# ap229997/hands

Hardware: AMD Instinct MI355X
Metric: hands/sec (higher is better)
Workload: dtype f32; 1 GPU; hands_light ResNet-50 x3 + feature_conv + HMR + MANO, 224x224, bz=256 samples/GPU (512 hands, 768 trunk passes); per_gpu_batch=256, global_batch=256, parallelism=dp1, rccl_ranks=1, launched_by=direct, conv3x3_stride1=winograd_f4x4:stages1234

## Files before the change

hands_amd/csrc/conv_wino4.hip:

```cpp
#include <hip/hip_runtime.h>
#include <stdint.h>
#include <stdlib.h>
#include "hands_hip.h"
#include "common.h"

#ifdef W4_PROF
__device__ unsigned long long g_w4prof[512 * 2 * 64];
extern "C" int hands_debug_w4prof(void* dst, int clear) {
  hipDeviceSynchronize();
  if (dst) hipMemcpyFromSymbol(dst, HIP_SYMBOL(g_w4prof), sizeof(unsigned long long) * 512 * 2 * 64);
  if (clear) { static unsigned long long z[512 * 2 * 64]; hipMemcpyToSymbol(HIP_SYMBOL(g_w4prof), z, sizeof(z)); }
  return 0;
}
#define W4_STAMP(ROLE, IDX)                                                                          \
  do {                                                                                              \
    __builtin_amdgcn_sched_barrier(0);                                                              \
    if (lane == 0 && blockIdx.x < 512 && (IDX) < 64 && (wave == 0 || wave == 12))                   \
      g_w4prof[(blockIdx.x * 2 + (ROLE)) * 64 + (IDX)] = __builtin_amdgcn_s_memtime();              \
    __builtin_amdgcn_sched_barrier(0);                                                              \
  } while (0)
#else
#define W4_STAMP(ROLE, IDX) do {} while (0)
#endif

namespace {

typedef unsigned int u32x4 __attribute__((ext_vector_type(4)));
typedef __attribute__((address_space(3))) void lds_void_t;

struct Wino4Args {
  const float* __restrict__ in;
  const float* __restrict__ u;
  const float* __restrict__ bias;
  float* out;
  int B, H, W, Cin, Cout, nh, nw;
  int in_ps, out_ps, act;
  int nblk_m, nblk_n, nseg;
  int band;
  int rows;
  uint32_t nh_mul, nh_sh;
};

__device__ __forceinline__ int w4_fastdiv(int x, uint32_t mul, uint32_t sh) {
  return mul == 0 ? x : (int)(__umulhi((uint32_t)x, mul) >> sh);
}

__device__ __forceinline__ int w4_xcd_remap(int bid, int nwg) {
  const int q = nwg >> 3, r = nwg & 7;
  const int xcd = bid & 7, idx = bid >> 3;
  const int base = (xcd < r) ? xcd * (q + 1) : r * (q + 1) + (xcd - r) * q;
  return base + idx;
}

__device__ __forceinline__ float4 w4_f4(const u32x4& v) {
  return make_float4(__uint_as_float(v.x), __uint_as_float(v.y), __uint_as_float(v.z), __uint_as_float(v.w));
}
__device__ __forceinline__ float w4_e(const float4& v, int t) { return t == 0 ? v.x : (t == 1 ? v.y : (t == 2 ? v.z : v.w)); }

__device__ __forceinline__ void w4_dma16(__amdgpu_buffer_rsrc_t rsrc, char* dst, int voff, int soff) {
  __builtin_amdgcn_raw_ptr_buffer_load_lds(rsrc, (lds_void_t*)dst, 16, voff, soff, 0, 0);
}

__device__ __forceinline__ void w4_bt6(const float (&x)[6], float (&v)[6]) {
  const float a = fmaf(-4.f, x[2], x[4]);
  const float b = fmaf(-4.f, x[1], x[3]);
  const float c = x[4] - x[2];
  const float d = x[3] - x[1];
  v[0] = fmaf(4.f, x[0], fmaf(-5.f, x[2], x[4]));
  v[1] = a + b;
  v[2] = a - b;
  v[3] = fmaf(2.f, d, c);
  v[4] = fmaf(-2.f, d, c);
  v[5] = fmaf(4.f, x[1], fmaf(-5.f, x[3], x[5]));
}

template <int D, bool LINEAR>
struct W4Geom {
  static constexpr int PW = 4 * D + 2;
  static constexpr int PWP = (PW + 3) / 4 * 4;
  static constexpr int NR = LINEAR ? (D - 1 + 32 + D - 1) / D : 32 / D;
  static constexpr int ROW_BYTES = PWP * 32;
  static constexpr int SLOTS = NR * 6 * PWP * 2;
  static constexpr int PIECES = (SLOTS + 63) / 64;
  static constexpr int NJ = (PIECES + 3) / 4;
  static constexpr int PATCH_BYTES = PIECES * 1024;
};

constexpr int W4_VBUF = 36 * 1024;
constexpr int W4_PATCH_MAX = 36 * 1024;
constexpr long long W4_BAND_BYTES = 2560 * 1024;

template <int D, bool LINEAR, int VSH>
__device__ __forceinline__ void w4_output_pass(const Wino4Args& a, const char* lds, int wave, int lane, int nb, int R0, int s0, int tx0) {
  constexpr int VM = (1 << VSH) - 1;
  const int rd = wave >> 2, oj = wave & 3;
  const int otl = lane >> 1, ocq = lane & 1;
  const int oqq = s0 + otl;
  const int oRl = LINEAR ? oqq / D : otl / D, ocol = LINEAR ? oqq - oRl * D : otl - oRl * D;
  const int oV = R0 + oRl, oR = oV >> VSH, otx = tx0 + (oV & VM) * D + ocol;
  const int ob = w4_fastdiv(oR, a.nh_mul, a.nh_sh), oty = oR - ob * a.nh;
  if (!(oR < a.rows && otx < a.nw && 4 * otx + oj < a.W)) return;
  const int n_ch = nb * 32 + rd * 8 + ocq * 4;
  float* const o = a.out + (((size_t)ob * a.H + 4 * oty) * a.W + 4 * otx + oj) * (size_t)a.out_ps + n_ch;
  const char* sE = lds + rd * W4_VBUF + otl * 32 + ocq * 16;
  const float kq = oj == 0 ? 1.f : (oj == 1 ? 2.f : (oj == 2 ? 4.f : 8.f));
  const int pi = (oj == 0 ? 0 : (oj == 2 ? 2 : 1)) * 1024, qi = (oj == 0 || oj == 2 ? 3 : 4) * 1024;
  float4 y[4];
#pragma unroll
  for (int x6 = 0; x6 < 6; ++x6) {
    const char* eb = sE + x6 * 6 * 1024;
    const float4 p0 = *reinterpret_cast<const float4*>(eb + pi);
    const float4 q0 = *reinterpret_cast<const float4*>(eb + qi);
    float4 z = make_float4(fmaf(kq, q0.x, p0.x), fmaf(kq, q0.y, p0.y), fmaf(kq, q0.z, p0.z), fmaf(kq, q0.w, p0.w));
    if (oj == 3) {
      const float4 m5 = *reinterpret_cast<const float4*>(eb + 5 * 1024);
      z.x += m5.x; z.y += m5.y; z.z += m5.z; z.w += m5.w;
    }
#define W4_ACC(C)                                                                                    \
    if (x6 == 0) { y[0].C = z.C; }                                                                  \
    else if (x6 == 1) { y[0].C += z.C; y[1].C = z.C; y[2].C = z.C; y[3].C = z.C; }                  \
    else if (x6 == 2) { y[0].C += z.C; y[1].C -= z.C; y[2].C += z.C; y[3].C -= z.C; }               \
    else if (x6 == 3) { y[0].C += z.C; y[1].C = fmaf(2.f, z.C, y[1].C); y[2].C = fmaf(4.f, z.C, y[2].C); y[3].C = fmaf(8.f, z.C, y[3].C); } \
    else if (x6 == 4) { y[0].C += z.C; y[1].C = fmaf(-2.f, z.C, y[1].C); y[2].C = fmaf(4.f, z.C, y[2].C); y[3].C = fmaf(-8.f, z.C, y[3].C); } \
    else { y[3].C += z.C; }
    W4_ACC(x) W4_ACC(y) W4_ACC(z) W4_ACC(w)
#undef W4_ACC
  }
  const float4 bv = *reinterpret_cast<const float4*>(a.bias + n_ch);
#pragma unroll
  for (int i = 0; i < 4; ++i) {
    float4 v = make_float4(y[i].x + bv.x, y[i].y + bv.y, y[i].z + bv.z, y[i].w + bv.w);
    if (a.act == HANDS_ACT_RELU) {
      v.x = fmaxf(v.x, 0.f); v.y = fmaxf(v.y, 0.f); v.z = fmaxf(v.z, 0.f); v.w = fmaxf(v.w, 0.f);
    } else if (a.act == HANDS_ACT_LEAKY_RELU) {
      v.x = v.x > 0.f ? v.x : 0.01f * v.x; v.y = v.y > 0.f ? v.y : 0.01f * v.y;
      v.z = v.z > 0.f ? v.z : 0.01f * v.z; v.w = v.w > 0.f ? v.w : 0.01f * v.w;
    }
    if (4 * oty + i < a.H) *reinterpret_cast<float4*>(o + (size_t)i * a.W * a.out_ps) = v;
  }
}

template <int D, bool LINEAR, int VSH, int NOB>
__global__ void __launch_bounds__(1024, 1) conv_wino4_f32_kernel(Wino4Args a) {
  using G = W4Geom<D, LINEAR>;
  static_assert(G::PATCH_BYTES <= W4_PATCH_MAX, "patch buffer");
  static_assert(VSH == 0 || LINEAR, "virtual rows exist in the linear block order only");
  __shared__ __attribute__((aligned(1024))) char lds[4 * W4_VBUF];
  char* const sV = lds;
  char* const sP = lds + 2 * W4_VBUF;

  const int tid = threadIdx.x;
  const int lane = tid & 63;
  const int wave = __builtin_amdgcn_readfirstlane(tid >> 6);
  const bool producer = wave >= 12;
  const int l31 = lane & 31, half = lane >> 5;
  constexpr int VM = (1 << VSH) - 1;

  const int wg = w4_xcd_remap(blockIdx.x, a.nblk_m * a.nblk_n);
  int nbg, mb;
  {
    const int full = a.nblk_n / a.band, per = a.band * a.nblk_m;
    int bi = wg / per, r = wg - bi * per, bw = a.band;
    if (bi >= full) { bi = full; r = wg - full * per; bw = a.nblk_n - full * a.band; }
    mb = r / bw;
    nbg = bi * a.band + (r - mb * bw);
  }
  const int nb = nbg * NOB;
  int R0, s0, tx0;
  if constexpr (LINEAR) {
    const int t0 = mb * 32;
    R0 = t0 / D; s0 = t0 - R0 * D; tx0 = 0;
  } else {
    const int rb = mb / a.nseg, seg = mb - rb * a.nseg;
    R0 = rb * G::NR; s0 = 0; tx0 = seg * D;
  }
  const int R0r = R0 >> VSH;
  const int b_first = w4_fastdiv(R0r, a.nh_mul, a.nh_sh);
  const int ty_first = R0r - b_first * a.nh;
  const int nsteps = a.Cin >> 3;

  if (producer) {
    W4_STAMP(1, 0);
    const int pw = wave - 12;
    __builtin_amdgcn_s_setprio(2);
    const __amdgpu_buffer_rsrc_t x_rsrc = __builtin_amdgcn_make_buffer_rsrc(
        const_cast<float*>(a.in) + (size_t)b_first * a.H * a.W * a.in_ps, 0, (int)0x80000000u, 0x00020000);
    int f_off[G::NJ];
#pragma unroll
    for (int j = 0; j < G::NJ; ++j) {
      const int i = j * 4 + pw;
      const int S = i * 64 + lane;
      const int r = S / (G::PWP * 2), within = S - r * (G::PWP * 2);
      const int Rl = r / 6, ar = r - Rl * 6;
      const int xg = within >> 3, sl = within & 7;
      const int swz = (D * Rl + xg) & 3;
      const int sl2 = sl ^ (swz << 1);
      const int x = 4 * xg + (sl2 >> 1), q = sl2 & 1;
      const int V = R0 + Rl, Rr = V >> VSH, pv = V & VM;
      const int t = ty_first + (Rr - R0r);
      const int db = w4_fastdiv(t, a.nh_mul, a.nh_sh), ty = t - db * a.nh;
      const int hy = 4 * ty - 1 + ar, wx = 4 * (tx0 + pv * D) - 1 + x;
      const bool ok = i < G::PIECES && x < G::PW && Rr < a.rows && (unsigned)hy < (unsigned)a.H && (unsigned)wx < (unsigned)a.W;
      f_off[j] = ok ? (((db * a.H + hy) * a.W + wx) * a.in_ps + q * 4) * 4 : (int)0x80000000u;
      if (i < G::PIECES) w4_dma16(x_rsrc, sP + i * 1024, f_off[j], 0);
    }
#define W4_PFILL(PB, G_)                                                                             \
  do {                                                                                              \
    _Pragma("unroll") for (int j = 0; j < G::NJ; ++j) {                                             \
      if (j * 4 + pw < G::PIECES) w4_dma16(x_rsrc, sP + (PB) * W4_VBUF + (j * 4 + pw) * 1024, f_off[j], (G_) * 32); \
    }                                                                                               \
  } while (0)
    if (nsteps > 1) W4_PFILL(1, 1);
    int tb[6];
    {
      const int tl = pw * 8 + (lane >> 3), c = lane & 7;
      const int qq = s0 + tl;
      const int Rl = LINEAR ? qq / D : tl / D, col = LINEAR ? qq - Rl * D : tl - Rl * D;
      const int swz0 = (D * Rl + col) & 3, swz1 = (swz0 + 1) & 3;
      const int q = c >> 2, w = c & 3;
#pragma unroll
      for (int b = 0; b < 6; ++b) {
        const int grp8 = b < 4 ? col : col + 1;
        const int sl = (2 * (b & 3) + q) ^ ((b < 4 ? swz0 : swz1) << 1);
        tb[b] = Rl * 6 * G::ROW_BYTES + (grp8 * 8 + sl) * 16 + w * 4;
      }
    }
    const int vw_off = pw * 256 + lane * 4;

#define W4_TRANSFORM(PB, VB, NEXT_FILL)                                                              \
  do {                                                                                              \
    const char* pp = sP + (PB) * W4_VBUF;                                                           \
    float xx[6][6];                                                                                 \
    _Pragma("unroll") for (int b = 0; b < 6; ++b)                                                   \
      _Pragma("unroll") for (int ar = 0; ar < 6; ++ar)                                              \
        xx[ar][b] = *reinterpret_cast<const float*>(pp + tb[b] + ar * G::ROW_BYTES);                \
    __builtin_amdgcn_sched_barrier(0);                                                              \
    NEXT_FILL;                                   \
    __builtin_amdgcn_sched_barrier(0);                                                              \
    float tt[6][6];                                                                                 \
    _Pragma("unroll") for (int b = 0; b < 6; ++b) {                                                 \
      float x[6], v[6];                                                                             \
      _Pragma("unroll") for (int ar = 0; ar < 6; ++ar) x[ar] = xx[ar][b];                           \
      w4_bt6(x, v);                                                                                 \
      _Pragma("unroll") for (int k = 0; k < 6; ++k) tt[k][b] = v[k];                                \
    }                                                                                               \
    char* vp = sV + (VB) * W4_VBUF + vw_off;                                                        \
    _Pragma("unroll") for (int k = 0; k < 6; ++k) {                                                 \
      float v[6];                                                                                   \
      w4_bt6(tt[k], v);                                                                             \
      _Pragma("unroll") for (int n = 0; n < 6; ++n) *reinterpret_cast<float*>(vp + (k * 6 + n) * 1024) = v[n]; \
    }                                                                                               \
  } while (0)

    __syncthreads();
    W4_TRANSFORM(0, 0, );
    __syncthreads();
    W4_STAMP(1, 1);
    for (int g = 0; g < nsteps; ++g) {
      W4_STAMP(1, 2 + 3 * g);
#if !(defined(W4_ABL) && W4_ABL == 2)
#if defined(W4_ABL) && W4_ABL == 5
      if (g + 1 < nsteps && (g & 2) == 0) {
#else
      if (g + 1 < nsteps) {
#endif
        if ((g & 1) == 0) W4_TRANSFORM(1, 1, if (g + 2 < nsteps) W4_PFILL(0, g + 2)); else W4_TRANSFORM(0, 0, if (g + 2 < nsteps) W4_PFILL(1, g + 2));
      }
#endif
      W4_STAMP(1, 3 + 3 * g);
      __syncthreads();
      W4_STAMP(1, 4 + 3 * g);
    }
#undef W4_TRANSFORM
#undef W4_PFILL
  }
  if (!producer) {
    W4_STAMP(0, 0);
    const int xi = wave >> 1, hh = wave & 1;
    const int f0 = xi * 6 + 3 * hh;
    const __amdgpu_buffer_rsrc_t w_rsrc = __builtin_amdgcn_make_buffer_rsrc(
        const_cast<float*>(a.u) + (size_t)nb * nsteps * 9216, 0, (int)0x80000000u, 0x00020000);
    const __amdgpu_buffer_rsrc_t w_rsrc1 = __builtin_amdgcn_make_buffer_rsrc(
        const_cast<float*>(a.u) + (size_t)(nb + NOB - 1) * nsteps * 9216, 0, (int)0x80000000u, 0x00020000);
    const int w_off = f0 * 1024 + lane * 16;
    const int v_off = f0 * 1024 + l31 * 32 + half * 16;
    f32x16 acc[3][NOB];
#pragma unroll
    for (int n = 0; n < 3; ++n)
#pragma unroll
      for (int o = 0; o < NOB; ++o)
#pragma unroll
        for (int r = 0; r < 16; ++r) acc[n][o][r] = 0.f;

    float4 wq[2][NOB], vq[2];
#define W4_LOADOP(SET, N, STEP, VP)                                                                  \
  do {                                                                                              \
    vq[SET] = *reinterpret_cast<const float4*>((VP) + (N) * 1024);                                  \
    wq[SET][0] = w4_f4(__builtin_amdgcn_raw_buffer_load_b128(w_rsrc, w_off + (N) * 1024, (STEP) * 36864, 0)); \
    if (NOB > 1) wq[SET][NOB - 1] = w4_f4(__builtin_amdgcn_raw_buffer_load_b128(w_rsrc1, w_off + (N) * 1024, (STEP) * 36864, 0)); \
  } while (0)
#define W4_LOADW(SET, N, STEP)                                                                       \
  do {                                                                                              \
    wq[SET][0] = w4_f4(__builtin_amdgcn_raw_buffer_load_b128(w_rsrc, w_off + (N) * 1024, (STEP) * 36864, 0)); \
    if (NOB > 1) wq[SET][NOB - 1] = w4_f4(__builtin_amdgcn_raw_buffer_load_b128(w_rsrc1, w_off + (N) * 1024, (STEP) * 36864, 0)); \
  } while (0)
#if defined(W4_ABL) && W4_ABL == 4
#define W4_NMFMA 1
#else
#define W4_NMFMA 4
#endif
#define W4_MFMAS(SET, N)                                                                             \
  do {                                                                                              \
    _Pragma("unroll") for (int o = 0; o < NOB; ++o)                                                 \
      _Pragma("unroll") for (int t = 0; t < W4_NMFMA; ++t)                                          \
        acc[N][o] = __builtin_amdgcn_mfma_f32_32x32x2f32(w4_e(wq[SET][o], t), w4_e(vq[SET], t), acc[N][o], 0, 0, 0); \
  } while (0)

#define W4_BARRIER() do { asm volatile("s_waitcnt lgkmcnt(0)\n\ts_barrier" ::: "memory"); } while (0)
    if constexpr (NOB == 2) {
#define W4_V2(N, VP) do { vq[0] = *reinterpret_cast<const float4*>((VP) + (N) * 1024); } while (0)
#define W4_MFMAS2(WSET, N)                                                                           \
  do {                                                                                              \
    _Pragma("unroll") for (int o = 0; o < NOB; ++o)                                                 \
      _Pragma("unroll") for (int t = 0; t < 4; ++t)                                                 \
        acc[N][o] = __builtin_amdgcn_mfma_f32_32x32x2f32(w4_e(wq[WSET][o], t), w4_e(vq[0], t), acc[N][o], 0, 0, 0); \
  } while (0)
      W4_LOADW(0, 0, 0);
      W4_BARRIER();
      W4_BARRIER();
      W4_STAMP(0, 1);
      for (int g = 0; g < nsteps; ++g) {
        const int gn = g + 1 < nsteps ? g + 1 : g;
        const char* vp = sV + (g & 1) * W4_VBUF + v_off;
        W4_V2(0, vp); W4_LOADW(1, 1, g);
        __builtin_amdgcn_sched_barrier(0);
        W4_MFMAS2(0, 0);
        __builtin_amdgcn_sched_barrier(0);
        W4_LOADW(0, 2, g);
        W4_V2(1, vp);
        __builtin_amdgcn_sched_barrier(0);
        W4_MFMAS2(1, 1);
        __builtin_amdgcn_sched_barrier(0);
        W4_V2(2, vp);
        __builtin_amdgcn_sched_barrier(0);
        W4_MFMAS2(0, 2);
        __builtin_amdgcn_sched_barrier(0);
        W4_LOADW(0, 0, gn);
        __builtin_amdgcn_sched_barrier(0);
        W4_STAMP(0, 2 + 3 * g);
        W4_BARRIER();
        W4_STAMP(0, 4 + 3 * g);
      }
#undef W4_MFMAS2
#undef W4_V2
    } else {
    W4_LOADW(0, 0, 0);
    W4_BARRIER();
    W4_BARRIER();
    W4_STAMP(0, 1);
    vq[0] = *reinterpret_cast<const float4*>(sV + v_off);
    for (int g = 0; g < nsteps; ++g) {
      const int gn = g + 1 < nsteps ? g + 1 : g;
      const char* vp = sV + (g & 1) * W4_VBUF + v_off;
      W4_LOADOP(1, 1, g, vp);
      __builtin_amdgcn_sched_barrier(0);
      W4_MFMAS(0, 0);
      __builtin_amdgcn_sched_barrier(0);
      W4_LOADOP(0, 2, g, vp);
      __builtin_amdgcn_sched_barrier(0);
      W4_MFMAS(1, 1);
      __builtin_amdgcn_sched_barrier(0);
      W4_LOADW(1, 0, gn);
      __builtin_amdgcn_sched_barrier(0);
      W4_MFMAS(0, 2);
      __builtin_amdgcn_sched_barrier(0);
      W4_STAMP(0, 2 + 3 * g);
      W4_BARRIER();
      W4_STAMP(0, 4 + 3 * g);
      {
        const char* vn = sV + ((g + 1) & 1) * W4_VBUF + v_off;
        vq[1] = *reinterpret_cast<const float4*>(vn);
      }
      if (++g >= nsteps) break;
      const int gn2 = g + 1 < nsteps ? g + 1 : g;
      const char* vp2 = sV + (g & 1) * W4_VBUF + v_off;
      W4_LOADOP(0, 1, g, vp2);
      __builtin_amdgcn_sched_barrier(0);
      W4_MFMAS(1, 0);
      __builtin_amdgcn_sched_barrier(0);
      W4_LOADOP(1, 2, g, vp2);
      __builtin_amdgcn_sched_barrier(0);
      W4_MFMAS(0, 1);
      __builtin_amdgcn_sched_barrier(0);
      W4_LOADW(0, 0, gn2);
      __builtin_amdgcn_sched_barrier(0);
      W4_MFMAS(1, 2);
      __builtin_amdgcn_sched_barrier(0);
      W4_STAMP(0, 2 + 3 * g);
      W4_BARRIER();
      W4_STAMP(0, 4 + 3 * g);
      vq[0] = *reinterpret_cast<const float4*>(sV + ((g + 1) & 1) * W4_VBUF + v_off);
    }
    }
#undef W4_BARRIER
#undef W4_LOADOP
#undef W4_LOADW
#undef W4_MFMAS

#define W4_LDS_BARRIER() do { asm volatile("s_waitcnt lgkmcnt(0)\n\ts_barrier" ::: "memory"); } while (0)
#pragma unroll
    for (int o = 0; o < NOB; ++o) {
      if (hh == 0) {
#pragma unroll
        for (int r = 0; r < 16; ++r) {
          const float s_ = acc[1][o][r] + acc[2][o][r], d_ = acc[1][o][r] - acc[2][o][r];
          acc[0][o][r] = acc[0][o][r] + s_; acc[1][o][r] = d_; acc[2][o][r] = s_;
        }
      } else {
#pragma unroll
        for (int r = 0; r < 16; ++r) {
          const float s_ = acc[0][o][r] + acc[1][o][r], d_ = acc[0][o][r] - acc[1][o][r];
          acc[0][o][r] = s_; acc[1][o][r] = d_;
        }
      }
      if (o > 0) W4_LDS_BARRIER();
#pragma unroll
      for (int rd = 0; rd < 4; ++rd)
#pragma unroll
        for (int n = 0; n < 3; ++n)
          *reinterpret_cast<float4*>(lds + rd * W4_VBUF + v_off + n * 1024) =
              make_float4(acc[n][o][4 * rd + 0], acc[n][o][4 * rd + 1], acc[n][o][4 * rd + 2], acc[n][o][4 * rd + 3]);
      if (NOB > 1) W4_LDS_BARRIER(); else __syncthreads();
      W4_STAMP(0, 60);
      w4_output_pass<D, LINEAR, VSH>(a, lds, wave, lane, nb + o, R0, s0, tx0);
    }
    W4_STAMP(0, 61);
    return;
  }
#pragma unroll
  for (int o = 0; o < NOB; ++o) {
    if (o > 0) W4_LDS_BARRIER();
    if (NOB > 1) W4_LDS_BARRIER(); else __syncthreads();
    W4_STAMP(1, 60);
    w4_output_pass<D, LINEAR, VSH>(a, lds, wave, lane, nb + o, R0, s0, tx0);
  }
  W4_STAMP(1, 61);
}

}

static void w4_magic(int d, uint32_t& mul, uint32_t& sh) {
  if (d <= 1) { mul = 0; sh = 0; return; }
  int l = 0;
  while ((1LL << l) < d) ++l;
  mul = (uint32_t)(((1ULL << (31 + l)) + (uint64_t)d - 1) / (uint64_t)d);
  sh = (uint32_t)(l - 1);
}

static long long w4_blocks(long long rows, int nw) {
  if (nw == 7 || nw == 14) return (rows * nw + 31) / 32;
  if (nw <= 2) return (rows + 15) / 16;
  return (rows + 7) / 8 * ((nw + 3) / 4);
}

template <int D, bool LINEAR, int VSH, int NOB>
static int w4_launch_nob(Wino4Args& a, hipStream_t stream) {
  using G = W4Geom<D, LINEAR>;
  const long long rows = a.rows;
  long long nblk_m;
  if (LINEAR) {
    nblk_m = (rows * (D << VSH) + 31) / 32;
    a.nseg = 1;
  } else {
    a.nseg = (a.nw + D - 1) / D;
    nblk_m = (rows + G::NR - 1) / G::NR * a.nseg;
  }
  a.nblk_n = a.Cout / (32 * NOB);
  {
    const long long wbytes = (long long)(a.Cin / 8) * 36864 * NOB;
    long long band = W4_BAND_BYTES / wbytes;
#ifdef HANDS_W4_BAND_ENV
    const char* env = getenv("HANDS_W4_BAND");
    if (env && atoi(env) > 0) band = atoi(env);
#endif
    a.band = (int)(band < 1 ? 1 : (band > a.nblk_n ? a.nblk_n : band));
  }
  if (nblk_m <= 0 || nblk_m * a.nblk_n > 0x7fffffffLL) return HANDS_EINVAL;
  a.nblk_m = (int)nblk_m;
  const long long nwg = nblk_m * a.nblk_n;
  w4_magic(a.nh, a.nh_mul, a.nh_sh);
  const long long imgs = G::NR / a.nh + 2;
  if (imgs * a.H * a.W * a.in_ps * 4 >= 0x7fffffffLL) return HANDS_EINVAL;
  hipLaunchKernelGGL((conv_wino4_f32_kernel<D, LINEAR, VSH, NOB>), dim3((unsigned)nwg), dim3(1024), 0, stream, a);
  return (int)hipGetLastError();
}

template <int D, bool LINEAR, int VSH = 0>
static int w4_launch(Wino4Args& a, hipStream_t stream) {
#ifndef HANDS_W4_NOB1
  if (a.Cout % 64 == 0) return w4_launch_nob<D, LINEAR, VSH, 2>(a, stream);
#endif
  return w4_launch_nob<D, LINEAR, VSH, 1>(a, stream);
}

static bool w4_ok(const hands_conv_desc* d) {
  if (d->B <= 0 || d->H <= 0 || d->W <= 0) return false;
  const int act = d->act & HANDS_ACT_MASK;
  const long long nh = (d->H + 3) / 4, nw = (d->W + 3) / 4, rows = (long long)d->B * nh;
  if (rows >= 0x7fffff00LL || rows * nw >= 0x7fffff00LL) return false;
  if (w4_blocks(rows, (int)nw) * (d->Cout / 32) > 0x7fffffffLL) return false;
  const long long ps = d->in_pix_stride > d->out_pix_stride ? d->in_pix_stride : d->out_pix_stride;
  if ((16 / nh + 2) * d->H * d->W * ps * 4 >= 0x7fffffffLL) return false;
  return d->KH == 3 && d->KW == 3 && d->stride == 1 && d->pad == 1 && d->Ho == d->H && d->Wo == d->W && d->Cin >= 16 &&
         d->Cin % 8 == 0 && d->Cout >= 32 && d->Cout % 32 == 0 && d->in_pix_stride >= d->Cin && d->out_pix_stride >= d->Cout &&
         d->in_pix_stride % 4 == 0 && d->out_pix_stride % 4 == 0 &&
         (act == HANDS_ACT_NONE || act == HANDS_ACT_RELU || act == HANDS_ACT_LEAKY_RELU) && !(d->act & HANDS_MATH_BF16X3);
}

extern "C" int hands_conv3x3_winograd4_supported(const hands_conv_desc* d) { return d && w4_ok(d) ? 1 : 0; }

extern "C" long long hands_conv3x3_winograd4_executed_macs(const hands_conv_desc* d) {
  if (!d || !w4_ok(d)) return 0;
  const long long nh = (d->H + 3) / 4, nw = (d->W + 3) / 4;
  return 36LL * w4_blocks((long long)d->B * nh, (int)nw) * 32 * d->Cin * d->Cout;
}

extern "C" int hands_conv3x3_winograd4_f32(const hands_conv_desc* d, const float* in, const float* u_packed, const float* bias,
                                           float* out, hands_stream_t stream) {
  if (!d || !in || !u_packed || !bias || !out || !w4_ok(d)) return HANDS_EINVAL;
  if ((((uintptr_t)in) | ((uintptr_t)u_packed) | ((uintptr_t)bias) | ((uintptr_t)out)) & 15) return HANDS_EINVAL;
  Wino4Args a;
  a.in = in; a.u = u_packed; a.bias = bias; a.out = out;
  a.B = d->B; a.H = d->H; a.W = d->W; a.Cin = d->Cin; a.Cout = d->Cout;
  a.nh = (d->H + 3) / 4; a.nw = (d->W + 3) / 4;
  a.in_ps = d->in_pix_stride; a.out_ps = d->out_pix_stride; a.act = d->act & HANDS_ACT_MASK;
  a.rows = d->B * a.nh;
  a.nblk_m = a.nblk_n = a.nseg = 0; a.band = 1;
  hipStream_t s = (hipStream_t)stream;
  if (a.nw == 7) return w4_launch<7, true>(a, s);
  if (a.nw == 14) return w4_launch<7, true, 1>(a, s);
  if (a.nw <= 2) return w4_launch<2, false>(a, s);
  return w4_launch<4, false>(a, s);
}
```

Baseline: 12090 hands/s.

## Spread Winograd F4 prologue patch DMA across all waves, use vmcnt-counted barriers

The initial input-patch loads for stage 0 are now issued by all 16 waves instead of only the 4 producer waves. The stage-1 prefetch is issued by the 12 consumer waves instead of the producers. The first two consumer barriers now wait on precise vmcnt counts, so the weight and stage-1 loads can stay in flight across the first barrier. Bias loads are hoisted ahead of the output-pass barriers, and the slot-offset math moves into a shared header. This is meant to shorten the prologue latency before the first MFMAs, at the cost of more complex wait accounting that could race if the counts are wrong.

```diff
diff --git a/hands_amd/csrc/conv_wino4.hip b/hands_amd/csrc/conv_wino4.hip
--- a/hands_amd/csrc/conv_wino4.hip
+++ b/hands_amd/csrc/conv_wino4.hip
@@ -3,6 +3,7 @@
 #include <stdlib.h>
 #include "hands_hip.h"
 #include "common.h"
+#include "wino4_slots.h"
 
 #ifdef W4_PROF
 __device__ unsigned long long g_w4prof[512 * 2 * 64];
@@ -22,6 +23,7 @@
 #else
 #define W4_STAMP(ROLE, IDX) do {} while (0)
 #endif
+#define W4_STAMP_G(ROLE, K, G_) do { if ((G_) < 12) W4_STAMP(ROLE, (K) + 3 * (G_)); } while (0)
 
 namespace {
 
@@ -41,10 +43,6 @@
   uint32_t nh_mul, nh_sh;
 };
 
-__device__ __forceinline__ int w4_fastdiv(int x, uint32_t mul, uint32_t sh) {
-  return mul == 0 ? x : (int)(__umulhi((uint32_t)x, mul) >> sh);
-}
-
 __device__ __forceinline__ int w4_xcd_remap(int bid, int nwg) {
   const int q = nwg >> 3, r = nwg & 7;
   const int xcd = bid & 7, idx = bid >> 3;
@@ -74,24 +72,17 @@
   v[5] = fmaf(4.f, x[1], fmaf(-5.f, x[3], x[5]));
 }
 
-template <int D, bool LINEAR>
-struct W4Geom {
-  static constexpr int PW = 4 * D + 2;
-  static constexpr int PWP = (PW + 3) / 4 * 4;
-  static constexpr int NR = LINEAR ? (D - 1 + 32 + D - 1) / D : 32 / D;
-  static constexpr int ROW_BYTES = PWP * 32;
-  static constexpr int SLOTS = NR * 6 * PWP * 2;
-  static constexpr int PIECES = (SLOTS + 63) / 64;
-  static constexpr int NJ = (PIECES + 3) / 4;
-  static constexpr int PATCH_BYTES = PIECES * 1024;
-};
-
 constexpr int W4_VBUF = 36 * 1024;
 constexpr int W4_PATCH_MAX = 36 * 1024;
 constexpr long long W4_BAND_BYTES = 2560 * 1024;
 
+__device__ __forceinline__ float4 w4_bias4(const Wino4Args& a, int wave, int lane, int nb) {
+  return *reinterpret_cast<const float4*>(a.bias + nb * 32 + (wave >> 2) * 8 + (lane & 1) * 4);
+}
+
 template <int D, bool LINEAR, int VSH>
-__device__ __forceinline__ void w4_output_pass(const Wino4Args& a, const char* lds, int wave, int lane, int nb, int R0, int s0, int tx0) {
+__device__ __forceinline__ void w4_output_pass(const Wino4Args& a, const char* lds, int wave, int lane, int nb, int R0, int s0, int tx0,
+                                               const float4& bv) {
   constexpr int VM = (1 << VSH) - 1;
   const int rd = wave >> 2, oj = wave & 3;
   const int otl = lane >> 1, ocq = lane & 1;
@@ -126,7 +117,6 @@
     W4_ACC(x) W4_ACC(y) W4_ACC(z) W4_ACC(w)
 #undef W4_ACC
   }
-  const float4 bv = *reinterpret_cast<const float4*>(a.bias + n_ch);
 #pragma unroll
   for (int i = 0; i < 4; ++i) {
     float4 v = make_float4(y[i].x + bv.x, y[i].y + bv.y, y[i].z + bv.z, y[i].w + bv.w);
@@ -154,7 +144,6 @@
   const int wave = __builtin_amdgcn_readfirstlane(tid >> 6);
   const bool producer = wave >= 12;
   const int l31 = lane & 31, half = lane >> 5;
-  constexpr int VM = (1 << VSH) - 1;
 
   const int wg = w4_xcd_remap(blockIdx.x, a.nblk_m * a.nblk_n);
   int nbg, mb;
@@ -167,50 +156,50 @@
   }
   const int nb = nbg * NOB;
   int R0, s0, tx0;
-  if constexpr (LINEAR) {
-    const int t0 = mb * 32;
-    R0 = t0 / D; s0 = t0 - R0 * D; tx0 = 0;
-  } else {
-    const int rb = mb / a.nseg, seg = mb - rb * a.nseg;
-    R0 = rb * G::NR; s0 = 0; tx0 = seg * D;
-  }
+  w4_block_origin<D, LINEAR>(mb, a.nseg, R0, s0, tx0);
   const int R0r = R0 >> VSH;
   const int b_first = w4_fastdiv(R0r, a.nh_mul, a.nh_sh);
   const int ty_first = R0r - b_first * a.nh;
   const int nsteps = a.Cin >> 3;
 
+  W4_STAMP(producer ? 1 : 0, 0);
+  if (producer) __builtin_amdgcn_s_setprio(2);
+  const __amdgpu_buffer_rsrc_t x_rsrc = __builtin_amdgcn_make_buffer_rsrc(
+      const_cast<float*>(a.in) + (size_t)b_first * a.H * a.W * a.in_ps, 0, (int)0x80000000u, 0x00020000);
+  W4Fill fill;
+  fill.H = a.H; fill.W = a.W; fill.in_ps = a.in_ps; fill.nh = a.nh; fill.rows = a.rows; fill.nh_mul = a.nh_mul; fill.nh_sh = a.nh_sh;
+  fill.R0 = R0; fill.R0r = R0r; fill.ty_first = ty_first; fill.tx0 = tx0;
+#pragma unroll
+  for (int k = 0; k < G::NK; ++k) {
+    const int i = w4_prologue_piece(wave, k);
+    if (i < G::PIECES) w4_dma16(x_rsrc, sP + i * 1024, w4_slot_src_offset<D, LINEAR, VSH>(i, lane, fill), 0);
+  }
+  __builtin_amdgcn_sched_barrier(0);
+#define W4_VM_BARRIER(N)                                                                             \
+  do {                                                                                              \
+    switch (N) {                                                 \
+      case 0: asm volatile("s_waitcnt vmcnt(0) lgkmcnt(0)\n\ts_barrier" ::: "memory"); break;       \
+      case 1: asm volatile("s_waitcnt vmcnt(1) lgkmcnt(0)\n\ts_barrier" ::: "memory"); break;       \
+      case 2: asm volatile("s_waitcnt vmcnt(2) lgkmcnt(0)\n\ts_barrier" ::: "memory"); break;       \
+      case 3: asm volatile("s_waitcnt vmcnt(3) lgkmcnt(0)\n\ts_barrier" ::: "memory"); break;       \
+      case 4: asm volatile("s_waitcnt vmcnt(4) lgkmcnt(0)\n\ts_barrier" ::: "memory"); break;       \
+      default: asm volatile("s_waitcnt vmcnt(5) lgkmcnt(0)\n\ts_barrier" ::: "memory"); break;      \
+    }                                                                                               \
+  } while (0)
+  static_assert(G::NK1 + 2 <= 5, "W4_VM_BARRIER covers 3 stage-1 pieces + 2 weight loads");
+
   if (producer) {
-    W4_STAMP(1, 0);
     const int pw = wave - 12;
-    __builtin_amdgcn_s_setprio(2);
-    const __amdgpu_buffer_rsrc_t x_rsrc = __builtin_amdgcn_make_buffer_rsrc(
-        const_cast<float*>(a.in) + (size_t)b_first * a.H * a.W * a.in_ps, 0, (int)0x80000000u, 0x00020000);
     int f_off[G::NJ];
 #pragma unroll
-    for (int j = 0; j < G::NJ; ++j) {
-      const int i = j * 4 + pw;
-      const int S = i * 64 + lane;
-      const int r = S / (G::PWP * 2), within = S - r * (G::PWP * 2);
-      const int Rl = r / 6, ar = r - Rl * 6;
-      const int xg = within >> 3, sl = within & 7;
-      const int swz = (D * Rl + xg) & 3;
-      const int sl2 = sl ^ (swz << 1);
-      const int x = 4 * xg + (sl2 >> 1), q = sl2 & 1;
-      const int V = R0 + Rl, Rr = V >> VSH, pv = V & VM;
-      const int t = ty_first + (Rr - R0r);
-      const int db = w4_fastdiv(t, a.nh_mul, a.nh_sh), ty = t - db * a.nh;
-      const int hy = 4 * ty - 1 + ar, wx = 4 * (tx0 + pv * D) - 1 + x;
-      const bool ok = i < G::PIECES && x < G::PW && Rr < a.rows && (unsigned)hy < (unsigned)a.H && (unsigned)wx < (unsigned)a.W;
-      f_off[j] = ok ? (((db * a.H + hy) * a.W + wx) * a.in_ps + q * 4) * 4 : (int)0x80000000u;
-      if (i < G::PIECES) w4_dma16(x_rsrc, sP + i * 1024, f_off[j], 0);
-    }
+    for (int j = 0; j < G::NJ; ++j) f_off[j] = w4_slot_src_offset<D, LINEAR, VSH>(w4_producer_piece(pw, j), lane, fill);
 #define W4_PFILL(PB, G_)                                                                             \
   do {                                                                                              \
     _Pragma("unroll") for (int j = 0; j < G::NJ; ++j) {                                             \
-      if (j * 4 + pw < G::PIECES) w4_dma16(x_rsrc, sP + (PB) * W4_VBUF + (j * 4 + pw) * 1024, f_off[j], (G_) * 32); \
+      const int i_ = w4_producer_piece(pw, j);                                                      \
+      if (i_ < G::PIECES) w4_dma16(x_rsrc, sP + (PB) * W4_VBUF + i_ * 1024, f_off[j], (G_) * 32);   \
     }                                                                                               \
   } while (0)
-    if (nsteps > 1) W4_PFILL(1, 1);
     int tb[6];
     {
       const int tl = pw * 8 + (lane >> 3), c = lane & 7;
@@ -226,6 +215,11 @@
       }
     }
     const int vw_off = pw * 256 + lane * 4;
+#pragma unroll
+    for (int j = 0; j < G::NJ; ++j) asm volatile("" : "+v"(f_off[j]));
+#pragma unroll
+    for (int b = 0; b < 6; ++b) asm volatile("" : "+v"(tb[b]));
+    W4_STAMP(1, 40);
 
 #define W4_TRANSFORM(PB, VB, NEXT_FILL)                                                              \
   do {                                                                                              \
@@ -253,11 +247,12 @@
   } while (0)
 
     __syncthreads();
+    W4_STAMP(1, 41);
     W4_TRANSFORM(0, 0, );
     __syncthreads();
     W4_STAMP(1, 1);
     for (int g = 0; g < nsteps; ++g) {
-      W4_STAMP(1, 2 + 3 * g);
+      W4_STAMP_G(1, 2, g);
 #if !(defined(W4_ABL) && W4_ABL == 2)
 #if defined(W4_ABL) && W4_ABL == 5
       if (g + 1 < nsteps && (g & 2) == 0) {
@@ -267,15 +262,24 @@
         if ((g & 1) == 0) W4_TRANSFORM(1, 1, if (g + 2 < nsteps) W4_PFILL(0, g + 2)); else W4_TRANSFORM(0, 0, if (g + 2 < nsteps) W4_PFILL(1, g + 2));
       }
 #endif
-      W4_STAMP(1, 3 + 3 * g);
+      W4_STAMP_G(1, 3, g);
       __syncthreads();
-      W4_STAMP(1, 4 + 3 * g);
+      W4_STAMP_G(1, 4, g);
     }
 #undef W4_TRANSFORM
 #undef W4_PFILL
   }
   if (!producer) {
-    W4_STAMP(0, 0);
+    const int n_st1 = nsteps > 1 ? (G::PIECES - 1 - wave) / 12 + 1 : 0;
+    if (nsteps > 1) {
+#pragma unroll
+      for (int k = 0; k < G::NK1; ++k) {
+        const int i = w4_prologue1_piece(wave, k);
+        if (i < G::PIECES) w4_dma16(x_rsrc, sP + W4_VBUF + i * 1024, w4_slot_src_offset<D, LINEAR, VSH>(i, lane, fill), 32);
+      }
+    }
+    __builtin_amdgcn_sched_barrier(0);
+    W4_STAMP(0, 40);
     const int xi = wave >> 1, hh = wave & 1;
     const int f0 = xi * 6 + 3 * hh;
     const __amdgpu_buffer_rsrc_t w_rsrc = __builtin_amdgcn_make_buffer_rsrc(
@@ -326,8 +330,10 @@
         acc[N][o] = __builtin_amdgcn_mfma_f32_32x32x2f32(w4_e(wq[WSET][o], t), w4_e(vq[0], t), acc[N][o], 0, 0, 0); \
   } while (0)
       W4_LOADW(0, 0, 0);
-      W4_BARRIER();
-      W4_BARRIER();
+      __builtin_amdgcn_sched_barrier(0);
+      W4_VM_BARRIER(n_st1 + NOB);
+      W4_STAMP(0, 41);
+      W4_VM_BARRIER(NOB);
       W4_STAMP(0, 1);
       for (int g = 0; g < nsteps; ++g) {
         const int gn = g + 1 < nsteps ? g + 1 : g;
@@ -347,16 +353,18 @@
         __builtin_amdgcn_sched_barrier(0);
         W4_LOADW(0, 0, gn);
         __builtin_amdgcn_sched_barrier(0);
-        W4_STAMP(0, 2 + 3 * g);
+        W4_STAMP_G(0, 2, g);
         W4_BARRIER();
-        W4_STAMP(0, 4 + 3 * g);
+        W4_STAMP_G(0, 4, g);
       }
 #undef W4_MFMAS2
 #undef W4_V2
     } else {
     W4_LOADW(0, 0, 0);
-    W4_BARRIER();
-    W4_BARRIER();
+    __builtin_amdgcn_sched_barrier(0);
+    W4_VM_BARRIER(n_st1 + NOB);
+    W4_STAMP(0, 41);
+    W4_VM_BARRIER(NOB);
     W4_STAMP(0, 1);
     vq[0] = *reinterpret_cast<const float4*>(sV + v_off);
     for (int g = 0; g < nsteps; ++g) {
@@ -374,9 +382,9 @@
       __builtin_amdgcn_sched_barrier(0);
       W4_MFMAS(0, 2);
       __builtin_amdgcn_sched_barrier(0);
-      W4_STAMP(0, 2 + 3 * g);
+      W4_STAMP_G(0, 2, g);
       W4_BARRIER();
-      W4_STAMP(0, 4 + 3 * g);
+      W4_STAMP_G(0, 4, g);
       {
         const char* vn = sV + ((g + 1) & 1) * W4_VBUF + v_off;
         vq[1] = *reinterpret_cast<const float4*>(vn);
@@ -396,9 +404,9 @@
       __builtin_amdgcn_sched_barrier(0);
       W4_MFMAS(1, 2);
       __builtin_amdgcn_sched_barrier(0);
-      W4_STAMP(0, 2 + 3 * g);
+      W4_STAMP_G(0, 2, g);
       W4_BARRIER();
-      W4_STAMP(0, 4 + 3 * g);
+      W4_STAMP_G(0, 4, g);
       vq[0] = *reinterpret_cast<const float4*>(sV + ((g + 1) & 1) * W4_VBUF + v_off);
     }
     }
@@ -410,19 +418,15 @@
 #define W4_LDS_BARRIER() do { asm volatile("s_waitcnt lgkmcnt(0)\n\ts_barrier" ::: "memory"); } while (0)
 #pragma unroll
     for (int o = 0; o < NOB; ++o) {
-      if (hh == 0) {
-#pragma unroll
-        for (int r = 0; r < 16; ++r) {
-          const float s_ = acc[1][o][r] + acc[2][o][r], d_ = acc[1][o][r] - acc[2][o][r];
-          acc[0][o][r] = acc[0][o][r] + s_; acc[1][o][r] = d_; acc[2][o][r] = s_;
-        }
-      } else {
-#pragma unroll
-        for (int r = 0; r < 16; ++r) {
-          const float s_ = acc[0][o][r] + acc[1][o][r], d_ = acc[0][o][r] - acc[1][o][r];
-          acc[0][o][r] = s_; acc[1][o][r] = d_;
-        }
+      const float4 bv = w4_bias4(a, wave, lane, nb + o);
+#pragma unroll
+      for (int r = 0; r < 16; ++r) {
+        const float x_ = hh == 0 ? acc[1][o][r] : acc[0][o][r], y_ = hh == 0 ? acc[2][o][r] : acc[1][o][r];
+        const float s_ = x_ + y_, d_ = x_ - y_;
+        const float p0 = hh == 0 ? acc[0][o][r] + s_ : s_, p2 = hh == 0 ? s_ : acc[2][o][r];
+        acc[0][o][r] = p0; acc[1][o][r] = d_; acc[2][o][r] = p2;
       }
+      W4_STAMP(0, 44 + 4 * o);
       if (o > 0) W4_LDS_BARRIER();
 #pragma unroll
       for (int rd = 0; rd < 4; ++rd)
@@ -430,31 +434,28 @@
         for (int n = 0; n < 3; ++n)
           *reinterpret_cast<float4*>(lds + rd * W4_VBUF + v_off + n * 1024) =
               make_float4(acc[n][o][4 * rd + 0], acc[n][o][4 * rd + 1], acc[n][o][4 * rd + 2], acc[n][o][4 * rd + 3]);
+      W4_STAMP(0, 45 + 4 * o);
       if (NOB > 1) W4_LDS_BARRIER(); else __syncthreads();
-      W4_STAMP(0, 60);
-      w4_output_pass<D, LINEAR, VSH>(a, lds, wave, lane, nb + o, R0, s0, tx0);
+      W4_STAMP(0, 46 + 4 * o);
+      w4_output_pass<D, LINEAR, VSH>(a, lds, wave, lane, nb + o, R0, s0, tx0, bv);
+      W4_STAMP(0, 47 + 4 * o);
     }
     W4_STAMP(0, 61);
     return;
   }
 #pragma unroll
   for (int o = 0; o < NOB; ++o) {
+    const float4 bv = w4_bias4(a, wave, lane, nb + o);
+    W4_STAMP(1, 45 + 4 * o);
     if (o > 0) W4_LDS_BARRIER();
     if (NOB > 1) W4_LDS_BARRIER(); else __syncthreads();
-    W4_STAMP(1, 60);
-    w4_output_pass<D, LINEAR, VSH>(a, lds, wave, lane, nb + o, R0, s0, tx0);
+    W4_STAMP(1, 46 + 4 * o);
+    w4_output_pass<D, LINEAR, VSH>(a, lds, wave, lane, nb + o, R0, s0, tx0, bv);
+    W4_STAMP(1, 47 + 4 * o);
   }
   W4_STAMP(1, 61);
 }
 
-}
-
-static void w4_magic(int d, uint32_t& mul, uint32_t& sh) {
-  if (d <= 1) { mul = 0; sh = 0; return; }
-  int l = 0;
-  while ((1LL << l) < d) ++l;
-  mul = (uint32_t)(((1ULL << (31 + l)) + (uint64_t)d - 1) / (uint64_t)d);
-  sh = (uint32_t)(l - 1);
 }
 
 static long long w4_blocks(long long rows, int nw) {
diff --git a/hands_amd/csrc/wino4_slots.h b/hands_amd/csrc/wino4_slots.h
--- /dev/null
+++ b/hands_amd/csrc/wino4_slots.h
@@ -0,0 +1,80 @@
+#pragma once
+#include <stdint.h>
+
+#if defined(__HIPCC__)
+#define W4_HD __host__ __device__ __forceinline__
+#else
+#define W4_HD inline
+#endif
+
+template <int D, bool LINEAR>
+struct W4Geom {
+  static constexpr int PW = 4 * D + 2;
+  static constexpr int PWP = (PW + 3) / 4 * 4;
+  static constexpr int NR = LINEAR ? (D - 1 + 32 + D - 1) / D : 32 / D;
+  static constexpr int ROW_BYTES = PWP * 32;
+  static constexpr int SLOTS = NR * 6 * PWP * 2;
+  static constexpr int PIECES = (SLOTS + 63) / 64;
+  static constexpr int NJ = (PIECES + 3) / 4;
+  static constexpr int NK = (PIECES + 15) / 16;
+  static constexpr int NK1 = (PIECES + 11) / 12;
+  static constexpr int PATCH_BYTES = PIECES * 1024;
+};
+
+W4_HD int w4_prologue_piece(int wave, int k) { return k * 16 + wave; }
+W4_HD int w4_prologue1_piece(int cw, int k) { return k * 12 + cw; }
+W4_HD int w4_producer_piece(int pw, int j) { return j * 4 + pw; }
+
+W4_HD int w4_fastdiv(int x, uint32_t mul, uint32_t sh) {
+#if defined(__HIP_DEVICE_COMPILE__)
+  return mul == 0 ? x : (int)(__umulhi((uint32_t)x, mul) >> sh);
+#else
+  return mul == 0 ? x : (int)((uint32_t)(((uint64_t)(uint32_t)x * mul) >> 32) >> sh);
+#endif
+}
+
+inline void w4_magic(int d, uint32_t& mul, uint32_t& sh) {
+  if (d <= 1) { mul = 0; sh = 0; return; }
+  int l = 0;
+  while ((1LL << l) < d) ++l;
+  mul = (uint32_t)(((1ULL << (31 + l)) + (uint64_t)d - 1) / (uint64_t)d);
+  sh = (uint32_t)(l - 1);
+}
+
+struct W4Fill {
+  int H, W, in_ps, nh, rows;
+  uint32_t nh_mul, nh_sh;
+  int R0, R0r, ty_first, tx0;
+};
+
+template <int D, bool LINEAR>
+W4_HD void w4_block_origin(int mb, int nseg, int& R0, int& s0, int& tx0) {
+  if (LINEAR) {
+    const int t0 = mb * 32;
+    R0 = t0 / D; s0 = t0 - R0 * D; tx0 = 0;
+  } else {
+    const int rb = mb / nseg, seg = mb - rb * nseg;
+    R0 = rb * W4Geom<D, LINEAR>::NR; s0 = 0; tx0 = seg * D;
+  }
+}
+
+constexpr int W4_OOR = (int)0x80000000u;
+
+template <int D, bool LINEAR, int VSH>
+W4_HD int w4_slot_src_offset(int piece, int lane, const W4Fill& f) {
+  using G = W4Geom<D, LINEAR>;
+  constexpr int VM = (1 << VSH) - 1;
+  const int S = piece * 64 + lane;
+  const int r = S / (G::PWP * 2), within = S - r * (G::PWP * 2);
+  const int Rl = r / 6, ar = r - Rl * 6;
+  const int xg = within >> 3, sl = within & 7;
+  const int swz = (D * Rl + xg) & 3;
+  const int sl2 = sl ^ (swz << 1);
+  const int x = 4 * xg + (sl2 >> 1), q = sl2 & 1;
+  const int V = f.R0 + Rl, Rr = V >> VSH, pv = V & VM;
+  const int t = f.ty_first + (Rr - f.R0r);
+  const int db = w4_fastdiv(t, f.nh_mul, f.nh_sh), ty = t - db * f.nh;
+  const int hy = 4 * ty - 1 + ar, wx = 4 * (f.tx0 + pv * D) - 1 + x;
+  const bool ok = piece < G::PIECES && x < G::PW && Rr < f.rows && (unsigned)hy < (unsigned)f.H && (unsigned)wx < (unsigned)f.W;
+  return ok ? (((db * f.H + hy) * f.W + wx) * f.in_ps + q * 4) * 4 : W4_OOR;
+}
```

Measured after the change: 12130 hands/s (median of 6 runs). Within noise of the previous version (+0.3%).
